# linebender/vello

Measured on AMD Instinct MI355X. Metric: frames/sec paris-30k 1600x1600 MSAA16; scenes/sec at 1/2/4/8 GPU, higher is better.
Workload: dtype f32+u32

## Files before the change

### vello_amd/csrc/engine/coarse.hip

```cpp
#include "engine.h"

namespace vk {

namespace {

constexpr uint32_t SUB_W = 8;
#ifndef VK_COARSE_NW
#define VK_COARSE_NW 8
#endif
constexpr uint32_t NW = VK_COARSE_NW;
constexpr uint32_t WG = 64 * NW;
constexpr uint32_t NB = 64 * NW;
constexpr uint32_t QCAP = 2 * NB;
static_assert((QCAP & (QCAP - 1u)) == 0u && QCAP >= NB - 1u + WG, "the queue is a ring of a power of two that holds a batch's leftovers and a round's arrivals");
constexpr uint32_t PART_CHUNK = 256;
constexpr uint32_t NONE = 0xffffffffu;
constexpr uint32_t EMIT_GROUP = 8;
constexpr uint32_t INITIAL_ROOM = PTCL_INITIAL_ALLOC - 1u - 2u - 1u;
constexpr uint32_t REGION_SLACK = 62u;
constexpr uint32_t KIND_NONE = 0u, KIND_PATH2 = 1u, KIND_PATH3 = 2u, KIND_BEGIN = 3u;

typedef unsigned long long u64;

struct __attribute__((packed, aligned(4))) PtclWords2 { uint32_t a, b; };
// ... 41 lines not shown
    if (k >= c) { k -= c; w >>= 4; pos += 4u; }
    c = (uint32_t)__popc(w & 3u);
    if (k >= c) { k -= c; w >>= 2; pos += 2u; }
    if (k >= (w & 1u)) pos += 1u;
    return pos;
}

__device__ __forceinline__ u64 transpose64(u64 x, uint32_t lane) {
    const u64 masks[6] = {0x00000000ffffffffull, 0x0000ffff0000ffffull, 0x00ff00ff00ff00ffull,
                          0x0f0f0f0f0f0f0f0full, 0x3333333333333333ull, 0x5555555555555555ull};
#pragma unroll
    for (uint32_t s = 0; s < 6u; s++) {
        const uint32_t j = 32u >> s;
        const u64 mask = masks[s];
        const uint32_t olo = (uint32_t)__shfl_xor((int)(uint32_t)x, (int)j), ohi = (uint32_t)__shfl_xor((int)(uint32_t)(x >> 32), (int)j);
        const u64 other = make64(olo, ohi);
        if ((lane & j) == 0u) x = (x & mask) | ((other & mask) << j);
        else x = (x & ~mask) | ((other & ~mask) >> j);
    }
    return x;
}

__device__ __forceinline__ uint32_t words_of(u64 m, u64 g, u64 k1, u64 k2, u64 k3) {
    return 3u * popc64(g) + 3u * popc64(m & k1) + 4u * popc64(m & k2) + popc64(m & k3);
}

__device__ __forceinline__ PtclWords2 plane_window(const uint32_t *__restrict__ bits, uint32_t b) {
    return *reinterpret_cast<const PtclWords2 *>(bits + (b >> 3));
}
__device__ __forceinline__ uint32_t window_bits(PtclWords2 w, uint32_t byte_shift, uint32_t b) {
    return (((w.a >> byte_shift) & 0xffu) | (((w.b >> byte_shift) & 0xffu) << 8)) >> (b & 7u);
}

}

__global__ void __launch_bounds__(256) k_coarse_prep(Config cfg, uint32_t n_el_blocks, const uint32_t *__restrict__ scene,
                                                     const DrawMonoid *__restrict__ draw_monoids, const uint32_t *__restrict__ info_bin_data,
                                                     const Path *__restrict__ paths, const Tile *__restrict__ tiles, const Bump *__restrict__ bump,
                                                     CoarseEl *__restrict__ coarse_el, uint32_t *__restrict__ tile_bits) {
    const uint32_t tid = threadIdx.x;
    if (blockIdx.x < n_el_blocks) {
        const uint32_t drawobj_ix = blockIdx.x * 256u + tid;
        if (drawobj_ix >= cfg.layout.n_draw_objects) return;
        CoarseEl e;
        e.tag = scene[cfg.layout.draw_tag_base + drawobj_ix];
        e.flags = 0u; e.w0 = 0u; e.dd = 0u; e.di = 0u; e.tiles = 0u; e.bbox_x = 0u; e.bbox_y = 0u;
        if (e.tag != DRAWTAG_NOP) {
            const DrawMonoid dm = draw_monoids[drawobj_ix];
            e.dd = cfg.layout.draw_data_base + dm.scene_offset;
            e.di = dm.info_offset;
            e.flags = info_bin_data[dm.info_offset];
            e.w0 = scene[e.dd];
            const Path path = paths[dm.path_ix];
            e.tiles = path.tiles;
            e.bbox_x = path.bbox[0] | (path.bbox[2] << 16);
            e.bbox_y = path.bbox[1] | (path.bbox[3] << 16);
        }
        coarse_el[drawobj_ix] = e;
        return;
    }
    const uint32_t n_tiles = minu(bump->tile, cfg.tiles_size);
    const uint32_t lane = tid & 63u;
    const uint32_t wave = (blockIdx.x - n_el_blocks) * 4u + (tid >> 6);
    const uint32_t n_waves = (gridDim.x - n_el_blocks) * 4u;
    for (uint32_t chunk = wave; chunk * 64u < n_tiles; chunk += n_waves) {
        const uint32_t i = chunk * 64u + lane;
        Tile t{1, 0u};
        if (i < n_tiles) t = tiles[i];
        const unsigned long long ms = __ballot(t.segment_count_or_ix != 0u);
        const unsigned long long mz = __ballot(t.backdrop == 0);
        const unsigned long long mo = __ballot((t.backdrop & 1) == 0);
        if (lane < 8u) {
            const uint32_t sh = 8u * lane;
            tile_bits[(size_t)chunk * 8u + lane] = ((uint32_t)(ms >> sh) & 0xffu) | (((uint32_t)(mz >> sh) & 0xffu) << 8) | (((uint32_t)(mo >> sh) & 0xffu) << 16);
        }
    }
}


__global__ void __launch_bounds__(WG) k_coarse(Config cfg, const uint32_t *__restrict__ scene, const BinHeader *__restrict__ bin_headers,
                                                const uint32_t *__restrict__ info_bin_data, const CoarseEl *__restrict__ coarse_el,
                                                const uint32_t *__restrict__ tile_bits, Tile *tiles, Bump *bump,
                                                uint32_t *ptcl, bool allow_cull, uint32_t *work_count, uint32_t *tile_order,
                                                SliceItem *slice_items, uint32_t *slice_counters, uint32_t slice_cap, uint32_t cov_cap,
                                                uint32_t slice_fills, uint32_t slice_min_fills) {
#ifdef VELLO_SIMT_EMU
    __shared__ CoarseLds sh;
#else
    extern __shared__ __attribute__((aligned(16))) unsigned char coarse_lds_raw[];
    CoarseLds &sh = *reinterpret_cast<CoarseLds *>(coarse_lds_raw);
#endif
    const uint32_t tid = threadIdx.x;
    const uint32_t lane = tid & 63u, wave = tid >> 6;
    {
        uint32_t failed = bump->failed & (STAGE_BINNING | STAGE_TILE_ALLOC | STAGE_FLATTEN | FAILED_SCENE);
        if (bump->seg_counts > cfg.seg_counts_size) failed |= STAGE_PATH_COUNT;
        if (failed != 0u) {
            if (blockIdx.x == 0 && tid == 0) atomicOr(&bump->failed, failed);
            return;
        }
    }
    const uint32_t width_in_bins = (cfg.width_in_tiles + N_TILE_X - 1u) / N_TILE_X;
    const uint32_t height_in_bins = (cfg.height_in_tiles + N_TILE_Y - 1u) / N_TILE_Y;
    const uint32_t n_bins = width_in_bins * height_in_bins;
    const uint32_t bin_ix = ((blockIdx.x >> 3) >> 2) * 8u + (blockIdx.x & 7u);
    const uint32_t quad = (blockIdx.x >> 3) & 3u;
    if (bin_ix >= n_bins) return;
    const uint32_t aligned_n_bins = (n_bins + N_TILE - 1u) & ~(N_TILE - 1u);
    const uint32_t n_partitions = (cfg.layout.n_draw_objects + N_TILE - 1u) / N_TILE;
    const uint32_t sub_x0 = N_TILE_X * (bin_ix % width_in_bins) + SUB_W * (quad & 1u);
    const uint32_t sub_y0 = N_TILE_Y * (bin_ix / width_in_bins) + SUB_W * (quad >> 1);
    const bool has_clips = cfg.layout.n_clips != 0u;
    const bool cull = allow_cull && !has_clips;
    const uint32_t ptcl_dyn_start = cfg.width_in_tiles * cfg.height_in_tiles * PTCL_INITIAL_ALLOC;
    if (tid == 0u) sh.seg_arrive = 0u;
#ifdef VELLO_COARSE_PROF
    long long prof_prev = clock64();
    uint32_t prof_acc[16] = {0u, 0u, 0u, 0u, 0u, 0u, 0u, 0u, 0u, 0u, 0u, 0u, 0u, 0u, 0u, 0u};
#define CPROF(k) do { const long long t_ = clock64(); prof_acc[k] += (uint32_t)(t_ - prof_prev); prof_prev = t_; } while (0)
#define CPROF_COUNT(k) prof_acc[k] += 1u
#else
#define CPROF(k)
#define CPROF_COUNT(k)
#endif

    const uint32_t this_tile_ix = (sub_y0 + lane / SUB_W) * cfg.width_in_tiles + sub_x0 + lane % SUB_W;
    const uint32_t blend_offset = this_tile_ix * PTCL_INITIAL_ALLOC;
    const uint32_t list_start = blend_offset + 1u;
    uint32_t cur = list_start;
    uint32_t room = INITIAL_ROOM;
    bool dead = false;
    uint32_t words_total = 0u;
    uint32_t fills_total = 0u;
    uint32_t clip_zero_depth = 0u, clip_depth = 0u, render_blend_depth = 0u, max_blend_depth = 0u;

    uint32_t partition_ix = 0u;
    uint32_t chunk_total = 0u, chunk_pos = 0u;
    auto refill = [&]() {
        __syncthreads();
        if (wave == 0u) {
            uint32_t carry = 0u;
#pragma unroll
            for (uint32_t k = 0; k < PART_CHUNK / 64u; k++) {
                const uint32_t p = partition_ix + k * 64u + lane;
                uint32_t count = 0u, off = 0u;
                if (p < n_partitions) {
                    const BinHeader bh = bin_headers[(size_t)p * aligned_n_bins + bin_ix];
                    count = bh.element_count;
                    off = bh.chunk_offset;
                }
                const uint32_t incl = wave_incl_scan_u32(count, (int)lane) + carry;
                sh.part_end[k * 64u + lane] = incl;
                sh.part_off[k * 64u + lane] = off;
                carry = (uint32_t)__shfl((int)incl, 63);
            }
            if (lane == 0u) sh.bcast = carry;
        }
        __syncthreads();
        chunk_total = sh.bcast;
        chunk_pos = 0u;
        partition_ix += PART_CHUNK;
    };
    auto fetch_index = [&](uint32_t &d) -> bool {
        while (chunk_pos >= chunk_total && partition_ix < n_partitions) refill();
        const bool any = chunk_pos < chunk_total;
        const uint32_t ix = chunk_pos + tid;
        d = NONE;
        if (ix < chunk_total) {
            uint32_t part = 0u;
#pragma unroll
            for (uint32_t i = 0; i < 8u; i++) {
                const uint32_t probe = part + (128u >> i);
                if (ix >= sh.part_end[probe - 1u]) part = probe;
            }
            const uint32_t local = ix - (part > 0u ? sh.part_end[part - 1u] : 0u);
            d = info_bin_data[cfg.layout.bin_data_start + sh.part_off[part] + local];
        }
        chunk_pos = minu(chunk_pos + WG, chunk_total);
        return any;
    };

    uint32_t qh = 0u, qlen = 0u;
    auto load_el = [&](uint32_t d) -> CoarseEl {
        CoarseEl e;
        e.tag = DRAWTAG_NOP;
        e.flags = 0u; e.w0 = 0u; e.dd = 0u; e.di = 0u; e.tiles = 0u; e.bbox_x = 0u; e.bbox_y = 0u;
        if (d != NONE) {
            const uint4 *p = reinterpret_cast<const uint4 *>(coarse_el + d);
            const uint4 a = p[0], b = p[1];
            e.tag = a.x; e.flags = a.y; e.w0 = a.z; e.dd = a.w;
            e.di = b.x; e.tiles = b.y; e.bbox_x = b.z; e.bbox_y = b.w;
        }
        return e;
    };
    uint32_t d_next;
    bool cur_valid = fetch_index(d_next);
    CoarseEl el_next = load_el(d_next);
    bool next_valid = cur_valid ? fetch_index(d_next) : false;
    bool more = cur_valid;
    while (cur_valid || qlen > 0u) {
        if (cur_valid) {
            const CoarseEl el = el_next;
            if (next_valid) el_next = load_el(d_next);
            const bool nn_valid = next_valid ? fetch_index(d_next) : false;
            cur_valid = next_valid;
            next_valid = nn_valid;
            more = cur_valid;
            CPROF(8);
            const int32_t bx0 = (int32_t)(el.bbox_x & 0xffffu), bx1 = (int32_t)(el.bbox_x >> 16);
            const int32_t by0 = (int32_t)(el.bbox_y & 0xffffu), by1 = (int32_t)(el.bbox_y >> 16);
            const int32_t dx = bx0 - (int32_t)sub_x0, dy = by0 - (int32_t)sub_y0;
            const int32_t x0 = clampi(dx, 0, (int32_t)SUB_W), y0 = clampi(dy, 0, (int32_t)SUB_W);
            const int32_t x1 = clampi(bx1 - (int32_t)sub_x0, 0, (int32_t)SUB_W), y1 = clampi(by1 - (int32_t)sub_y0, 0, (int32_t)SUB_W);
            const bool meets = el.tag != DRAWTAG_NOP && x1 > x0 && y1 > y0;
            const uint32_t stride = (uint32_t)(bx1 - bx0);
            const uint32_t base = el.tiles - (uint32_t)(dy * (int32_t)stride + dx);
            u64 inc = 0ull, kil = 0ull, seg = 0ull, clr = 0ull;
            {
                const uint32_t rx0 = (uint32_t)x0, ry0 = (uint32_t)y0;
                const uint32_t w = meets ? (uint32_t)(x1 - x0) : 0u, h = meets ? (uint32_t)(y1 - y0) : 0u;
                const bool is_clip = (el.tag & 1u) != 0u;
                const uint32_t BLEND_CLIP = (128u << 8) | 3u;
                const bool is_blend = is_clip && el.w0 != BLEND_CLIP;
                const bool even_odd = (el.flags & DRAW_INFO_FLAGS_FILL_RULE_BIT) != 0u;
                const uint32_t clear_byte = even_odd ? 16u : 8u;
                const uint32_t wmask = (1u << w) - 1u;
                const uint32_t b0 = base + stride * ry0 + rx0;
                PtclWords2 win[SUB_W];
#pragma unroll
                for (uint32_t r = 0; r < SUB_W; r++) win[r] = plane_window(tile_bits, r < h ? b0 + stride * r : 0u);
#pragma unroll
                for (uint32_t r = 0; r < SUB_W; r++) {
                    const uint32_t rmask = r < h ? wmask : 0u;
                    const uint32_t b = b0 + stride * r;
                    const uint32_t sg = window_bits(win[r], 0u, b) & rmask;
                    const uint32_t clear = window_bits(win[r], clear_byte, b) & rmask;
                    const uint32_t in = is_blend ? rmask : (sg | ((is_clip ? clear : ~clear) & rmask));
                    const uint32_t shift = ((ry0 + r) * SUB_W + rx0) & 63u;
                    inc |= (u64)in << shift;
                    seg |= (u64)(in & sg) << shift;
                    clr |= (u64)(in & clear) << shift;
                }
                if (cull && el.tag == DRAWTAG_FILL_COLOR && (el.w0 >> 24) == 0xffu) kil = inc & ~seg;
            }
            const bool keep = inc != 0ull;
            const u64 m = __ballot(keep);
            CPROF(9);
            if (lane == 0u) sh.wave_cnt[wave] = popc64(m);
            __syncthreads();
            CPROF(10);
            uint32_t before = 0u, total_new = 0u;
#pragma unroll
            for (uint32_t w = 0; w < NW; w++) {
                const uint32_t c = sh.wave_cnt[w];
                if (w < wave) before += c;
                total_new += c;
            }
            if (keep) {
                const uint32_t q = (qh + qlen + before + popc64(m & below64(lane))) & (QCAP - 1u);
                uint32_t kind = KIND_NONE;
                switch (el.tag) {
                case DRAWTAG_FILL_COLOR: case DRAWTAG_FILL_IMAGE: kind = KIND_PATH2; break;
                case DRAWTAG_BLURRED_ROUNDED_RECT: case DRAWTAG_FILL_LIN_GRADIENT: case DRAWTAG_FILL_RAD_GRADIENT:
                case DRAWTAG_FILL_SWEEP_GRADIENT: case DRAWTAG_END_CLIP: kind = KIND_PATH3; break;
                case DRAWTAG_BEGIN_CLIP: kind = KIND_BEGIN; break;
                default: break;
                }
                sh.tag[q] = el.tag;
                sh.flags[q] = el.flags;
                sh.w0[q] = el.w0;
                sh.dd[q] = el.dd;
                sh.di[q] = el.di;
                sh.stride[q] = stride;
                sh.base[q] = base;
                sh.kind[q] = kind;
                sh.cover[q][0] = (uint32_t)inc; sh.cover[q][1] = (uint32_t)(inc >> 32);
                sh.cover[q][2] = (uint32_t)kil; sh.cover[q][3] = (uint32_t)(kil >> 32);
                sh.cover[q][4] = (uint32_t)seg; sh.cover[q][5] = (uint32_t)(seg >> 32);
                sh.cover[q][6] = (uint32_t)clr; sh.cover[q][7] = (uint32_t)(clr >> 32);
            }
            qlen += total_new;
            __syncthreads();
            CPROF(0);
            CPROF_COUNT(6);
        }

        while (qlen >= NB || (!more && qlen > 0u)) {
            const uint32_t n = minu(qlen, NB);
            const uint32_t cnt = n > wave * 64u ? minu(n - wave * 64u, 64u) : 0u;
            const uint32_t q0 = qh + wave * 64u;
            const uint32_t my_kind = lane < cnt ? (sh.kind[(q0 + lane) & (QCAP - 1u)]) : KIND_NONE;
            const u64 k1 = __ballot(my_kind == KIND_PATH2), k2 = __ballot(my_kind == KIND_PATH3), k3 = __ballot(my_kind == KIND_BEGIN);
            const u64 k_end = has_clips ? __ballot(lane < cnt && sh.tag[(q0 + lane) & (QCAP - 1u)] == DRAWTAG_END_CLIP) : 0ull;
            u64 inc = 0ull, seg = 0ull, clr = 0ull, kil = 0ull;
            if (lane < cnt) {
                const uint32_t *c = sh.cover[(q0 + lane) & (QCAP - 1u)];
                inc = make64(c[0], c[1]);
                if (cull) kil = make64(c[2], c[3]);
                seg = make64(c[4], c[5]);
                if (has_clips) clr = make64(c[6], c[7]);
            }
            inc = transpose64(inc, lane);
            seg = transpose64(seg, lane);
            if (cull) kil = transpose64(kil, lane);
            if (has_clips) clr = transpose64(clr, lane);
            const uint32_t klast = kil != 0ull ? 64u - (uint32_t)__clzll((long long)kil) : 0u;
            sh.kslice[wave][lane] = klast;
            if (has_clips) {
                sh.em[wave][lane][0] = (uint32_t)inc; sh.em[wave][lane][1] = (uint32_t)(inc >> 32);
                sh.gm[wave][lane][0] = (uint32_t)seg; sh.gm[wave][lane][1] = (uint32_t)(seg >> 32);
                sh.cl[wave][lane][0] = (uint32_t)clr; sh.cl[wave][lane][1] = (uint32_t)(clr >> 32);
                if (lane == 0u) {
                    sh.kinds[wave][0][0] = (uint32_t)k3; sh.kinds[wave][0][1] = (uint32_t)(k3 >> 32);
                    sh.kinds[wave][1][0] = (uint32_t)k_end; sh.kinds[wave][1][1] = (uint32_t)(k_end >> 32);
                }
            }
            __syncthreads();
            bool tile_killed = false;
            if (cull) {
                bool later = false;
#pragma unroll
                for (uint32_t w = 0; w < NW; w++) {
                    const uint32_t kl = sh.kslice[w][lane];
                    tile_killed = tile_killed || kl != 0u;
                    if (w > wave && kl != 0u) later = true;
                }
                if (later) inc = 0ull;
                else if (klast != 0u) inc &= ~below64(klast - 1u);
            }
            if (has_clips) {
                if (wave == 0u) {
#pragma unroll 1
                    for (uint32_t w = 0; w < NW; w++) {
                        const u64 m = make64(sh.em[w][lane][0], sh.em[w][lane][1]);
                        const u64 sg = make64(sh.gm[w][lane][0], sh.gm[w][lane][1]);
                        const u64 cr = make64(sh.cl[w][lane][0], sh.cl[w][lane][1]);
                        const u64 kb = make64(sh.kinds[w][0][0], sh.kinds[w][0][1]);
                        const u64 ke = make64(sh.kinds[w][1][0], sh.kinds[w][1][1]);
                        u64 clipbits = m & (kb | ke);
                        u64 act = 0ull;
// ... 41 lines not shown
            const u64 gmask = seg & em & (k1 | k2);
            const uint32_t n_pairs_t = popc64(em);
            const uint32_t pair_incl = wave_incl_scan_u32(n_pairs_t, (int)lane);
            const uint32_t total_pairs = (uint32_t)__shfl((int)pair_incl, 63);
            sh.em[wave][lane][0] = (uint32_t)em; sh.em[wave][lane][1] = (uint32_t)(em >> 32);
            sh.gm[wave][lane][0] = (uint32_t)gmask; sh.gm[wave][lane][1] = (uint32_t)(gmask >> 32);
            sh.pend[wave][lane] = pair_incl;
            sh.S[wave][lane] = words_of(em, gmask, k1, k2, k3) | (popc64(gmask) << 16);
            wave_lds_sync();
            const uint32_t n_iter = (total_pairs + 63u) / 64u;
            auto pair_of = [&](uint32_t p, uint32_t &t, uint32_t &b, bool &has_segs) {
                t = 0u;
#pragma unroll
                for (uint32_t i = 0; i < 6u; i++) {
                    const uint32_t probe = t + (32u >> i);
                    if (p >= sh.pend[wave][probe - 1u]) t = probe;
                }
                const uint32_t k = p - (t > 0u ? sh.pend[wave][t - 1u] : 0u);
                const u64 m = make64(sh.em[wave][t][0], sh.em[wave][t][1]);
                b = kth_bit64(m, k);
                has_segs = ((make64(sh.gm[wave][t][0], sh.gm[wave][t][1]) >> b) & 1ull) != 0ull;
            };
            auto load_group = [&](uint32_t g0, uint32_t (&info)[EMIT_GROUP], uint32_t (&tix)[EMIT_GROUP], Tile (&tl)[EMIT_GROUP]) {
#pragma unroll
                for (uint32_t u = 0; u < EMIT_GROUP; u++) {
                    const uint32_t p = (g0 + u) * 64u + lane;
                    info[u] = 0u;
                    tix[u] = 0u;
                    tl[u] = Tile{0, 0u};
                    if (g0 + u < n_iter && p < total_pairs) {
                        uint32_t t, b;
                        bool has_segs;
                        pair_of(p, t, b, has_segs);
                        const uint32_t q = (q0 + b) & (QCAP - 1u);
                        tix[u] = sh.base[q] + sh.stride[q] * (t / SUB_W) + (t % SUB_W);
                        info[u] = t | (b << 8) | (has_segs ? 1u << 16 : 0u) | (1u << 17);
                        if (has_segs) tl[u] = tiles[tix[u]];
                    }
                }
            };
            uint32_t info[EMIT_GROUP], tix[EMIT_GROUP];
            Tile tl[EMIT_GROUP];
            load_group(0u, info, tix, tl);
            __syncthreads();
            CPROF(1);
            if (wave == 0u) {
                uint32_t s_w[NW], W = 0u, n_fill = 0u;
#pragma unroll
                for (uint32_t w = 0; w < NW; w++) {
                    const uint32_t s = sh.S[w][lane];
                    s_w[w] = s & 0xffffu;
                    W += s_w[w];
                    n_fill += s >> 16;
                }
                if (tile_killed && !dead) {
                    cur = list_start;
                    room = INITIAL_ROOM;
                    words_total = 0u;
                    fills_total = 0u;
                }
                words_total += W;
                fills_total += n_fill;
                const bool need = W > room && !dead;
                const uint32_t rsize = need ? W + 2u + REGION_SLACK : 0u;
                const uint32_t r_incl = wave_incl_scan_u32(rsize, (int)lane);
                const uint32_t r_total = (uint32_t)__shfl((int)r_incl, 63);
                uint32_t r_base = 0u;
                if (lane == 0u && r_total != 0u) r_base = atomicAdd(&bump->ptcl, r_total);
                r_base = (uint32_t)__shfl((int)r_base, 0);
                if (need) {
                    const uint32_t start = ptcl_dyn_start + r_base + (r_incl - rsize);
                    if (start < ptcl_dyn_start || start + rsize > cfg.ptcl_size || start + rsize < start) {
                        atomicOr(&bump->failed, STAGE_COARSE);
                        dead = true;
                    } else {
                        *reinterpret_cast<PtclWords2 *>(ptcl + cur) = PtclWords2{CMD_JUMP, start};
                        cur = start;
                        room = W + REGION_SLACK;
                    }
                }
                uint32_t wb = dead ? NONE : cur;
#pragma unroll
                for (uint32_t w = 0; w < NW; w++) {
                    sh.wordbase[w][lane] = wb;
                    if (!dead) wb += s_w[w];
                }
                if (!dead) {
                    cur += W;
                    room -= W;
                }
            }
            CPROF(2);
            uint32_t seg_first;
            {
                uint32_t my_segs = 0u;
#pragma unroll
                for (uint32_t u = 0; u < EMIT_GROUP; u++) my_segs += tl[u].segment_count_or_ix;
                const uint32_t seg_incl = wave_incl_scan_u32(my_segs, (int)lane);
                const uint32_t seg_total = (uint32_t)__shfl((int)seg_incl, 63);
                uint32_t arrived = 0u;
                if (lane == 0u) {
                    sh.seg_tot[wave] = seg_total;
#ifdef VELLO_SIMT_EMU
                    arrived = atomicAdd(&sh.seg_arrive, 1u);
#else
                    arrived = __hip_atomic_fetch_add(&sh.seg_arrive, 1u, __ATOMIC_ACQ_REL, __HIP_MEMORY_SCOPE_WORKGROUP);
#endif
                }
                arrived = (uint32_t)__shfl((int)arrived, 0);
                if (arrived == NW - 1u) {
                    const uint32_t tot = lane < NW ? sh.seg_tot[lane] : 0u;
                    const uint32_t incl = wave_incl_scan_u32(tot, (int)lane);
                    const uint32_t all = (uint32_t)__shfl((int)incl, 63);
                    uint32_t got = 0u;
                    if (lane == 0u && all != 0u) got = atomicAdd(&bump->segments, all);
                    got = (uint32_t)__shfl((int)got, 0);
                    if (lane < NW) sh.seg_base[lane] = got + (incl - tot);
                    if (lane == 0u) sh.seg_arrive = 0u;
                }
                __syncthreads();
                seg_first = sh.seg_base[wave] + (seg_incl - my_segs);
            }
            for (uint32_t g0 = 0; g0 < n_iter; g0 += EMIT_GROUP) {
                uint32_t seg_next = seg_first;
                if (g0 != 0u) {
                    load_group(g0, info, tix, tl);
                    uint32_t my_segs = 0u;
#pragma unroll
                    for (uint32_t u = 0; u < EMIT_GROUP; u++) my_segs += tl[u].segment_count_or_ix;
                    const uint32_t seg_incl = wave_incl_scan_u32(my_segs, (int)lane);
                    const uint32_t seg_total = (uint32_t)__shfl((int)seg_incl, 63);
                    uint32_t got = 0u;
                    if (lane == 0u && seg_total != 0u) got = atomicAdd(&bump->segments, seg_total);
                    seg_next = (uint32_t)__shfl((int)got, 0) + (seg_incl - my_segs);
                }
#pragma unroll
                for (uint32_t u = 0; u < EMIT_GROUP; u++) {
                    if ((info[u] >> 17) == 0u) continue;
                    const uint32_t t = info[u] & 0xffu, b = (info[u] >> 8) & 0xffu;
                    const bool has_segs = ((info[u] >> 16) & 1u) != 0u;
                    const uint32_t n_segs = tl[u].segment_count_or_ix;
                    const uint32_t seg_ix = seg_next;
                    seg_next += n_segs;
                    const uint32_t wbase = sh.wordbase[wave][t];
                    if (wbase == NONE) continue;
                    const uint32_t q = (q0 + b) & (QCAP - 1u);
                    const u64 m = make64(sh.em[wave][t][0], sh.em[wave][t][1]);
                    const u64 g = make64(sh.gm[wave][t][0], sh.gm[wave][t][1]);
                    const u64 bel = below64(b);
                    uint32_t off = wbase + words_of(m & bel, g & bel, k1, k2, k3);
                    const uint32_t tag = sh.tag[q];
                    if (tag == DRAWTAG_BEGIN_CLIP) {
                        ptcl[off] = CMD_BEGIN_CLIP;
                        continue;
                    }
                    const uint32_t draw_flags = sh.flags[q];
                    if (has_segs) {
                        tiles[tix[u]].segment_count_or_ix = ~seg_ix;
                        const uint32_t even_odd = (draw_flags & DRAW_INFO_FLAGS_FILL_RULE_BIT) != 0u ? 1u : 0u;
                        *reinterpret_cast<PtclWords4 *>(ptcl + off) = PtclWords4{CMD_FILL, (n_segs << 1) | even_odd, seg_ix, (uint32_t)tl[u].backdrop};
                        off += 4u;
                    } else {
                        ptcl[off] = CMD_SOLID;
                        off += 1u;
                    }
                    const uint32_t w0 = sh.w0[q], di = sh.di[q];
                    switch (tag) {
                    case DRAWTAG_FILL_COLOR: *reinterpret_cast<PtclWords2 *>(ptcl + off) = PtclWords2{CMD_COLOR, w0}; break;
                    case DRAWTAG_FILL_IMAGE: *reinterpret_cast<PtclWords2 *>(ptcl + off) = PtclWords2{CMD_IMAGE, di + 1u}; break;
                    case DRAWTAG_BLURRED_ROUNDED_RECT: *reinterpret_cast<PtclWords3 *>(ptcl + off) = PtclWords3{CMD_BLUR_RECT, di + 1u, w0}; break;
                    case DRAWTAG_FILL_LIN_GRADIENT: *reinterpret_cast<PtclWords3 *>(ptcl + off) = PtclWords3{CMD_LIN_GRAD, w0, di + 1u}; break;
                    case DRAWTAG_FILL_RAD_GRADIENT: *reinterpret_cast<PtclWords3 *>(ptcl + off) = PtclWords3{CMD_RAD_GRAD, w0, di + 1u}; break;
                    case DRAWTAG_FILL_SWEEP_GRADIENT: *reinterpret_cast<PtclWords3 *>(ptcl + off) = PtclWords3{CMD_SWEEP_GRAD, w0, di + 1u}; break;
                    case DRAWTAG_END_CLIP: *reinterpret_cast<PtclWords3 *>(ptcl + off) = PtclWords3{CMD_END_CLIP, w0, scene[sh.dd[q] + 1u]}; break;
                    default: break;
                    }
                }
            }
            CPROF(3);
            qh = (qh + n) & (QCAP - 1u);
            qlen -= n;
            __syncthreads();
            CPROF(4);
            CPROF_COUNT(7);
        }
    }
    if (wave == 0u) {
        const bool in_target = sub_x0 + lane % SUB_W < cfg.width_in_tiles && sub_y0 + lane / SUB_W < cfg.height_in_tiles;
        if (in_target) {
            if (!dead) ptcl[cur] = CMD_END;
            uint32_t blend_ix = 0u;
            if (max_blend_depth > BLEND_STACK_SPLIT) {
                uint32_t scratch_size = (max_blend_depth - BLEND_STACK_SPLIT) * TILE_WIDTH * TILE_HEIGHT;
                blend_ix = atomicAdd(&bump->blend, scratch_size);
                if (blend_ix + scratch_size > cfg.blend_size) atomicOr(&bump->failed, STAGE_COARSE);
            }
            ptcl[blend_offset] = blend_ix;
            ptcl[blend_offset + PTCL_INITIAL_ALLOC - 1u] = words_total;
        }
        const uint32_t n_tiles = cfg.width_in_tiles * cfg.height_in_tiles;
        uint32_t bucket = in_target ? minu(FINE_WORK_BUCKETS - 1u, words_total / FINE_BUCKET_WORDS) : NONE;
        uint32_t n_sl = 0u;
        if (in_target && !dead && slice_min_fills != 0u && fills_total >= slice_min_fills) n_sl = minu((fills_total + slice_fills - 1u) / slice_fills, 0xffffu);
        if (__ballot(n_sl != 0u) != 0ull) {
            const uint32_t cov_need = n_sl != 0u ? n_sl * slice_fills * 64u + 64u : 0u;
            const uint32_t it_incl = wave_incl_scan_u32(n_sl, (int)lane), cv_incl = wave_incl_scan_u32(cov_need, (int)lane);
            uint32_t it_base = 0u, cv_base = 0u;
            if (lane == 63u) {
                it_base = atomicAdd(&work_count[FINE_WORK_BUCKETS], it_incl);
                cv_base = atomicAdd(&work_count[FINE_WORK_BUCKETS + 1u], cv_incl);
            }
            it_base = (uint32_t)__shfl((int)it_base, 63) + (it_incl - n_sl);
            cv_base = (uint32_t)__shfl((int)cv_base, 63) + (cv_incl - cov_need);
            if (n_sl != 0u) {
                const bool fits = it_base + n_sl <= slice_cap && it_base + n_sl >= it_base && cv_base + cov_need <= cov_cap && cv_base + cov_need >= cv_base;
                for (uint32_t k = 0; k < n_sl && it_base + k < slice_cap && it_base + k >= it_base; k++)
                    slice_items[it_base + k] = SliceItem{fits ? this_tile_ix : ~0u, k | (n_sl << 16), cv_base, it_base};
                if (fits) {
                    slice_counters[it_base] = 0u;
                    bucket = NONE;
                }
            }
        }
        static_assert(FINE_WORK_BUCKETS <= 64u, "a lane per bucket");
        uint32_t my_count = 0u, my_rank = 0u;
        for (uint32_t bk = 0; bk < FINE_WORK_BUCKETS; bk++) {
            const u64 m = __ballot(bucket == bk);
            if (lane == bk) my_count = popc64(m);
            if (bucket == bk) my_rank = popc64(m & below64(lane));
        }
        uint32_t base = 0u;
        if (lane < FINE_WORK_BUCKETS && my_count != 0u) base = atomicAdd(&work_count[lane], my_count);
        base = (uint32_t)__shfl((int)base, (int)(bucket & 63u));
        if (bucket != NONE) {
            const uint32_t pos = base + my_rank;
            if (pos < n_tiles) tile_order[bucket * n_tiles + pos] = this_tile_ix;
        }
    }
#ifdef VELLO_COARSE_PROF
    CPROF(5);
    if (tid == 0u && cfg.ptcl_size >= 8192u && blockIdx.x < 512u)
        for (uint32_t k = 0; k < 16u; k++) ptcl[cfg.ptcl_size - 8192u + blockIdx.x * 16u + k] = prof_acc[k];
#endif
}

int enable_coarse_lds() {
#ifndef VELLO_SIMT_EMU
    return (int)hipFuncSetAttribute(reinterpret_cast<const void *>(k_coarse), hipFuncAttributeMaxDynamicSharedMemorySize, (int)sizeof(CoarseLds));
#else
    return 0;
#endif
}

constexpr uint32_t COARSE_GRID_BINS = 8u;
uint32_t coarse_batch_draws() { return NB; }
uint32_t coarse_grid_bins() { return COARSE_GRID_BINS; }

void launch_coarse(const Frame &f, hipStream_t s, hipEvent_t *mid) {
    const uint32_t wb = (f.cfg.width_in_tiles + 15u) / 16u, hb = (f.cfg.height_in_tiles + 15u) / 16u;
    if (wb * hb == 0) {
        if (mid) (void)hipEventRecord(mid[0], s);
        return;
    }
    const uint32_t n_el_blocks = (f.cfg.layout.n_draw_objects + DRAW_WG - 1u) / DRAW_WG;
    uint32_t n_bit_blocks = (uint32_t)(((uint64_t)f.cfg.tiles_size + 256u * 8u - 1u) / (256u * 8u));
    if (n_bit_blocks > 2048u) n_bit_blocks = 2048u;
    if (n_bit_blocks < 1u) n_bit_blocks = 1u;
    hipLaunchKernelGGL(k_coarse_prep, dim3(n_el_blocks + n_bit_blocks), dim3(256), 0, s, dd_config(f), n_el_blocks, f.scene, f.draw_monoids,
                       f.info_bin_data, f.paths, f.tiles, f.bump(), f.coarse_el, f.tile_bits);
    if (mid) (void)hipEventRecord(mid[0], s);
    const uint32_t n_wg = ((wb * hb + COARSE_GRID_BINS - 1u) / COARSE_GRID_BINS) * COARSE_GRID_BINS * 4u;
    hipLaunchKernelGGL(k_coarse, dim3(n_wg), dim3(WG), sizeof(CoarseLds), s, f.cfg, f.scene, f.bin_headers, f.info_bin_data, f.coarse_el, f.tile_bits,
                       f.tiles, f.bump(), f.ptcl, !f.no_cull, f.control->work_count, f.tile_order,
                       f.slice_items, f.slice_counters, f.slice_cap, f.cov_cap, f.slice_fills, f.slice_min_fills);
}

}
```

### vello_amd/csrc/engine/engine.h

```cpp
#pragma once
#include <cstddef>
#include "common.h"

namespace vk {

constexpr uint32_t SCAN_STATUS_AGG = 1, SCAN_STATUS_PREFIX = 2;
constexpr uint32_t PATHTAG_PART_WORDS = 1024;
constexpr uint32_t DRAW_PART = 256;
constexpr uint32_t DRAW_WG = 256;
#ifndef VK_FLATTEN_TPT
#define VK_FLATTEN_TPT 4
#endif
constexpr uint32_t FLATTEN_TAGS_PER_THREAD = VK_FLATTEN_TPT;
constexpr uint32_t FLATTEN_BLOCK_TAGS = 256 * FLATTEN_TAGS_PER_THREAD;
#ifndef VK_PC_LPT
#define VK_PC_LPT 4
#endif
constexpr uint32_t PATH_COUNT_LINES_PER_THREAD = VK_PC_LPT;
constexpr uint32_t PATH_COUNT_CHUNK = 256 * PATH_COUNT_LINES_PER_THREAD;
constexpr int64_t PATH_COUNT_SMALL_MAX_LINES = 768 * 256;
constexpr uint32_t SPIN_LIMIT = 1u << 24;
constexpr uint32_t FAILED_INTERNAL = 0x80000000u;
constexpr uint32_t FAILED_SCENE = 0x40000000u;
constexpr uint32_t FINE_WORK_BUCKETS = 32;
// ... 15 lines not shown
#endif
constexpr uint32_t FINE_SLICE_FILLS_IN_FLIGHT = VK_SLICE_FILLS_IN_FLIGHT, FINE_SLICE_MIN_FILLS_IN_FLIGHT = VK_SLICE_MIN_FILLS_IN_FLIGHT;
constexpr uint32_t FINE_SLICE_FILLS_FORCED = 4, FINE_SLICE_MIN_FILLS_FORCED = 5;
struct SliceItem {
    uint32_t tile_ix;
    uint32_t k_and_n;
    uint32_t cov_base;
    uint32_t first_item;
};
constexpr uint32_t CLIP_PART = 256;
constexpr uint32_t CLIP_MAX_PARTS = 2048;
struct ClipEl { uint32_t clip_ix; float x0, y0, x1, y1; };
__host__ __device__ inline uint32_t clip_parts_pad(uint32_t parts) {
    uint32_t n = 2u;
    while (n < parts) n <<= 1;
    return n;
}
inline size_t clip_scratch_words(uint32_t n_clips) {
    size_t parts = (n_clips + CLIP_PART - 1u) / CLIP_PART;
    size_t par = parts * (CLIP_PART * 5u + 4u + 2u + 1u) + 2u * (size_t)clip_parts_pad((uint32_t)parts);
    size_t seq = ((size_t)n_clips + 1u) * 6u;
    return par > seq ? par : seq;
}

struct Control {
    Bump bump;
    uint32_t ticket_pathtag;
    uint32_t ticket_draw;
    uint32_t heavy_count[4];
    uint32_t pad[2];
    uint32_t work_count[FINE_WORK_BUCKETS];
    uint32_t slice_items;
    uint32_t cov_words;
    uint32_t pad2[48 - FINE_WORK_BUCKETS - 2];
    uint32_t arc_count[64];
};
static_assert(sizeof(Control) == 512, "Control");
static_assert(offsetof(Control, slice_items) == offsetof(Control, work_count) + 4u * FINE_WORK_BUCKETS, "Control::slice_items follows work_count");
static_assert(offsetof(Control, cov_words) == offsetof(Control, slice_items) + 4u, "Control::cov_words follows slice_items");
constexpr uint32_t FLATTEN_ARC_SHARDS = 64;
#ifndef VK_STROKES_GRID_SIDE_BY_SIDE
#define VK_STROKES_GRID_SIDE_BY_SIDE 4096u
#endif
#ifndef VK_STROKES_GRID_OWN_LAUNCH
#define VK_STROKES_GRID_OWN_LAUNCH 384u
#endif
inline uint32_t flatten_strokes_grid(uint32_t n_seg_max, bool side_by_side) {
    const uint32_t cap = side_by_side ? VK_STROKES_GRID_SIDE_BY_SIDE : VK_STROKES_GRID_OWN_LAUNCH;
    const uint32_t g = (n_seg_max + 255u) / 256u;
    return g > cap ? cap : (g < 1u ? 1u : g);
}
inline uint32_t flatten_arc_shard_cap(uint32_t n_seg_max, bool side_by_side) {
    const uint32_t grid = flatten_strokes_grid(n_seg_max, side_by_side);
    const uint32_t rounds = ((n_seg_max + 255u) / 256u + grid - 1u) / grid;
    return ((grid + FLATTEN_ARC_SHARDS - 1u) / FLATTEN_ARC_SHARDS) * (rounds < 1u ? 1u : rounds) * 256u;
}

struct Frame {
    Config cfg;
    uint32_t n_tag_words;
    uint32_t n_scene_words;
    uint32_t aa;
    const uint32_t *scene;
    uint32_t xf_base;
    bool has_view;
    Xform view;
    bool retained;
    const uint32_t *xf_owner;
    const uint32_t *pose_words;
    uint32_t n_instances;
    hipStream_t pose_stream;
    hipEvent_t pose_mark;
    bool pose_check;
// ... 233 lines not shown
```

### vello_amd/csrc/engine/fine.hip

```cpp
#include "engine.h"

namespace vk {

namespace {

constexpr uint32_t PIXELS_PER_THREAD = 4;
constexpr int GRADIENT_WIDTH = 512;
constexpr uint32_t LUMINANCE_MASK_LAYER = 0x10000u;

enum {
    FP_INTERP = 0,
    FP_BATCH_SCAN,
    FP_BATCH_SEGS,
    FP_BATCH_ITEMS,
    FP_FILL_APPLY,
    FP_FILL_PREFIX,
    FP_FILL_SPARSE,
    FP_FILL_RESTORE,
    FP_FILL_EVENODD,
    FP_FILL_UNBATCHED,
    FP_BLEND,
    FP_RARE,
    FP_RARE_END_CLIP,
    FP_RARE_GRAD,
// ... 1489 lines not shown
        slice_n = it.k_and_n >> 16;
        mode = MODE_COV;
        fill_lo = k * slice_fills;
        fill_hi = k + 1u == slice_n ? 0xffffffffu : (k + 1u) * slice_fills;
        fill_room = slice_n * slice_fills;
        cov_base = it.cov_base;
        first_item = it.first_item;
    } else {
        const uint32_t rest = blockIdx.x - (AA != 0 ? slice_blocks : 0u);
        static_assert(FINE_WORK_BUCKETS <= 64u, "a lane per bucket");
        const uint32_t cnt = lane < FINE_WORK_BUCKETS ? minu(work_count[FINE_WORK_BUCKETS - 1u - lane], n_tiles) : 0u;
        const uint32_t incl = wave_incl_scan_u32(cnt, (int)lane);
        const unsigned long long beyond = __ballot(incl > rest);
        if (beyond == 0ull) return;
        const uint32_t bl = (uint32_t)__ffsll((long long)beyond) - 1u;
        const uint32_t slot = (FINE_WORK_BUCKETS - 1u - bl) * n_tiles + (rest - wave_read(incl - cnt, bl));
        tile_ix = (uint32_t)__builtin_amdgcn_readfirstlane((int)tile_order[slot]);
        if (tile_ix >= n_tiles) return;
    }
    const uint32_t tile_x = tile_ix % cfg.width_in_tiles, tile_y = tile_ix / cfg.width_in_tiles;
    const float xy_x = (float)(tile_x * TILE_WIDTH + lx * PIXELS_PER_THREAD);
    const float xy_y = (float)(tile_y * TILE_HEIGHT + ly);
    vec4 rgba[4];
    uint32_t blend_stack[BLEND_STACK_SPLIT][4];
    uint32_t clip_depth;
    float area[4];
    uint32_t cmd_ix;
    uint32_t win_base;
    uint32_t win;
    auto rd = [&](uint32_t ix) -> uint32_t {
        return (uint32_t)__builtin_amdgcn_readlane((int)win, (int)__builtin_amdgcn_readfirstlane((int)(ix - win_base)));
    };
    auto ensure = [&](uint32_t ix, uint32_t n_words) {
        if (ix + n_words > win_base + FINE_WINDOW_WORDS) {
            win_base = ix;
            uint32_t a = win_base + lane;
            win = a < cfg.ptcl_size ? ptcl[a] : 0u;
        }
    };
    FineProf prof;
    prof.start();
    FineTimeline tl;
    tl.start();
    uint32_t blend_offset;
    constexpr float COV_SCALE = AA == 2 ? 0.0625f : 0.125f;
    uint32_t fill_no = 0u;
    auto start_list = [&]() {
        const vec4 base_color = unpack4x8unorm(cfg.base_color);
#pragma unroll
        for (int i = 0; i < 4; i++) {
            rgba[i] = base_color;
            area[i] = 0.0f;
        }
        clip_depth = 0u;
        cmd_ix = tile_ix * PTCL_INITIAL_ALLOC;
        win_base = cmd_ix;
        win = ptcl[win_base + lane];
        blend_offset = rd(cmd_ix);
        cmd_ix += 1u;
        fill_no = 0u;
    };
    auto store_cov = [&]() {
        uint32_t b = 0u;
#pragma unroll
        for (uint32_t i = 0; i < 4u; i++) b |= (uint32_t)(area[i] * (1.0f / COV_SCALE)) << (8u * i);
        if (fill_no < fill_room) __hip_atomic_store(&cov[cov_base + fill_no * 64u + lane], b, __ATOMIC_RELAXED, __HIP_MEMORY_SCOPE_AGENT);
        fill_no += 1u;
// ... 291 lines not shown
```

Measured before the change: 2673.

## Walk draw objects back-to-front in coarse to stop at opaque-covered tiles

Adds a back-to-front coarse mode, selected when culling is allowed, there are no clips, and the prep kernel flagged at least one opaque solid fill. Partitions and queue batches are processed in reverse order, and per-tile command lists are built backwards through prepended regions linked by jumps. Each tile stops once an opaque fill covers it, and the workgroup exits early once all its tiles are covered, so occluded draws are never binned or emitted. The cost is extra prep-kernel sync and flag writes, a templated second kernel path, and the fine window reloading on backward jumps. The chained, non-contiguous command lists may also hurt fine's read locality.

```diff
diff --git a/vello_amd/csrc/engine/coarse.hip b/vello_amd/csrc/engine/coarse.hip
--- a/vello_amd/csrc/engine/coarse.hip
+++ b/vello_amd/csrc/engine/coarse.hip
@@ -97,31 +97,42 @@
     return (((w.a >> byte_shift) & 0xffu) | (((w.b >> byte_shift) & 0xffu) << 8)) >> (b & 7u);
 }
 
+__device__ __forceinline__ bool coarse_back_to_front(bool allow_cull, uint32_t n_clips, bool opaque_fills) {
+    return allow_cull && n_clips == 0u && opaque_fills;
+}
+
 }
 
 __global__ void __launch_bounds__(256) k_coarse_prep(Config cfg, uint32_t n_el_blocks, const uint32_t *__restrict__ scene,
                                                      const DrawMonoid *__restrict__ draw_monoids, const uint32_t *__restrict__ info_bin_data,
                                                      const Path *__restrict__ paths, const Tile *__restrict__ tiles, const Bump *__restrict__ bump,
-                                                     CoarseEl *__restrict__ coarse_el, uint32_t *__restrict__ tile_bits) {
+                                                     CoarseEl *__restrict__ coarse_el, uint32_t *__restrict__ tile_bits, uint32_t *opaque_fills) {
     const uint32_t tid = threadIdx.x;
     if (blockIdx.x < n_el_blocks) {
+        __shared__ uint32_t any_opaque;
+        if (tid == 0u) any_opaque = 0u;
+        __syncthreads();
         const uint32_t drawobj_ix = blockIdx.x * 256u + tid;
-        if (drawobj_ix >= cfg.layout.n_draw_objects) return;
-        CoarseEl e;
-        e.tag = scene[cfg.layout.draw_tag_base + drawobj_ix];
-        e.flags = 0u; e.w0 = 0u; e.dd = 0u; e.di = 0u; e.tiles = 0u; e.bbox_x = 0u; e.bbox_y = 0u;
-        if (e.tag != DRAWTAG_NOP) {
-            const DrawMonoid dm = draw_monoids[drawobj_ix];
-            e.dd = cfg.layout.draw_data_base + dm.scene_offset;
-            e.di = dm.info_offset;
-            e.flags = info_bin_data[dm.info_offset];
-            e.w0 = scene[e.dd];
-            const Path path = paths[dm.path_ix];
-            e.tiles = path.tiles;
-            e.bbox_x = path.bbox[0] | (path.bbox[2] << 16);
-            e.bbox_y = path.bbox[1] | (path.bbox[3] << 16);
-        }
-        coarse_el[drawobj_ix] = e;
+        if (drawobj_ix < cfg.layout.n_draw_objects) {
+            CoarseEl e;
+            e.tag = scene[cfg.layout.draw_tag_base + drawobj_ix];
+            e.flags = 0u; e.w0 = 0u; e.dd = 0u; e.di = 0u; e.tiles = 0u; e.bbox_x = 0u; e.bbox_y = 0u;
+            if (e.tag != DRAWTAG_NOP) {
+                const DrawMonoid dm = draw_monoids[drawobj_ix];
+                e.dd = cfg.layout.draw_data_base + dm.scene_offset;
+                e.di = dm.info_offset;
+                e.flags = info_bin_data[dm.info_offset];
+                e.w0 = scene[e.dd];
+                const Path path = paths[dm.path_ix];
+                e.tiles = path.tiles;
+                e.bbox_x = path.bbox[0] | (path.bbox[2] << 16);
+                e.bbox_y = path.bbox[1] | (path.bbox[3] << 16);
+            }
+            coarse_el[drawobj_ix] = e;
+            if (e.tag == DRAWTAG_FILL_COLOR && (e.w0 >> 24) == 0xffu) any_opaque = 1u;
+        }
+        __syncthreads();
+        if (tid == 0u && any_opaque != 0u) opaque_fills[blockIdx.x % COARSE_OPAQUE_SHARDS] = 1u;
         return;
     }
     const uint32_t n_tiles = minu(bump->tile, cfg.tiles_size);
@@ -143,18 +154,13 @@
 }
 
 
-__global__ void __launch_bounds__(WG) k_coarse(Config cfg, const uint32_t *__restrict__ scene, const BinHeader *__restrict__ bin_headers,
+template <bool B2F>
+__device__ __forceinline__ void coarse_workgroup(CoarseLds &sh, const Config &cfg, const uint32_t *__restrict__ scene, const BinHeader *__restrict__ bin_headers,
                                                 const uint32_t *__restrict__ info_bin_data, const CoarseEl *__restrict__ coarse_el,
                                                 const uint32_t *__restrict__ tile_bits, Tile *tiles, Bump *bump,
                                                 uint32_t *ptcl, bool allow_cull, uint32_t *work_count, uint32_t *tile_order,
                                                 SliceItem *slice_items, uint32_t *slice_counters, uint32_t slice_cap, uint32_t cov_cap,
                                                 uint32_t slice_fills, uint32_t slice_min_fills) {
-#ifdef VELLO_SIMT_EMU
-    __shared__ CoarseLds sh;
-#else
-    extern __shared__ __attribute__((aligned(16))) unsigned char coarse_lds_raw[];
-    CoarseLds &sh = *reinterpret_cast<CoarseLds *>(coarse_lds_raw);
-#endif
     const uint32_t tid = threadIdx.x;
     const uint32_t lane = tid & 63u, wave = tid >> 6;
     {
@@ -175,8 +181,8 @@
     const uint32_t n_partitions = (cfg.layout.n_draw_objects + N_TILE - 1u) / N_TILE;
     const uint32_t sub_x0 = N_TILE_X * (bin_ix % width_in_bins) + SUB_W * (quad & 1u);
     const uint32_t sub_y0 = N_TILE_Y * (bin_ix / width_in_bins) + SUB_W * (quad >> 1);
-    const bool has_clips = cfg.layout.n_clips != 0u;
-    const bool cull = allow_cull && !has_clips;
+    const bool has_clips = !B2F && cfg.layout.n_clips != 0u;
+    const bool cull = B2F || (allow_cull && !has_clips);
     const uint32_t ptcl_dyn_start = cfg.width_in_tiles * cfg.height_in_tiles * PTCL_INITIAL_ALLOC;
     if (tid == 0u) sh.seg_arrive = 0u;
 #ifdef VELLO_COARSE_PROF
@@ -198,11 +204,16 @@
     uint32_t words_total = 0u;
     uint32_t fills_total = 0u;
     uint32_t clip_zero_depth = 0u, clip_depth = 0u, render_blend_depth = 0u, max_blend_depth = 0u;
-
-    uint32_t partition_ix = 0u;
+    bool covered = B2F && !(sub_x0 + lane % SUB_W < cfg.width_in_tiles && sub_y0 + lane / SUB_W < cfg.height_in_tiles);
+    u64 covered_mask = B2F ? __ballot(covered) : 0ull;
+    uint32_t head = NONE, front = 0u;
+    bool finished = false;
+
+    uint32_t partition_ix = B2F ? ((n_partitions + PART_CHUNK - 1u) / PART_CHUNK) * PART_CHUNK : 0u;
     uint32_t chunk_total = 0u, chunk_pos = 0u;
     auto refill = [&]() {
         __syncthreads();
+        if (B2F) partition_ix -= PART_CHUNK;
         if (wave == 0u) {
             uint32_t carry = 0u;
 #pragma unroll
@@ -224,12 +235,12 @@
         __syncthreads();
         chunk_total = sh.bcast;
         chunk_pos = 0u;
-        partition_ix += PART_CHUNK;
+        if (!B2F) partition_ix += PART_CHUNK;
     };
     auto fetch_index = [&](uint32_t &d) -> bool {
-        while (chunk_pos >= chunk_total && partition_ix < n_partitions) refill();
+        while (chunk_pos >= chunk_total && (B2F ? partition_ix > 0u : partition_ix < n_partitions)) refill();
         const bool any = chunk_pos < chunk_total;
-        const uint32_t ix = chunk_pos + tid;
+        const uint32_t ix = B2F ? chunk_total - 1u - (chunk_pos + tid) : chunk_pos + tid;
         d = NONE;
         if (ix < chunk_total) {
             uint32_t part = 0u;
@@ -263,7 +274,8 @@
     CoarseEl el_next = load_el(d_next);
     bool next_valid = cur_valid ? fetch_index(d_next) : false;
     bool more = cur_valid;
-    while (cur_valid || qlen > 0u) {
+    bool all_covered = false;
+    while ((cur_valid || qlen > 0u) && !all_covered) {
         if (cur_valid) {
             const CoarseEl el = el_next;
             if (next_valid) el_next = load_el(d_next);
@@ -306,6 +318,7 @@
                     seg |= (u64)(in & sg) << shift;
                     clr |= (u64)(in & clear) << shift;
                 }
+                if (B2F) inc &= ~covered_mask;
                 if (cull && el.tag == DRAWTAG_FILL_COLOR && (el.w0 >> 24) == 0xffu) kil = inc & ~seg;
             }
             const bool keep = inc != 0ull;
@@ -353,13 +366,15 @@
         while (qlen >= NB || (!more && qlen > 0u)) {
             const uint32_t n = minu(qlen, NB);
             const uint32_t cnt = n > wave * 64u ? minu(n - wave * 64u, 64u) : 0u;
-            const uint32_t q0 = qh + wave * 64u;
-            const uint32_t my_kind = lane < cnt ? (sh.kind[(q0 + lane) & (QCAP - 1u)]) : KIND_NONE;
+            auto slot_q = [&](uint32_t j) -> uint32_t { return (B2F ? qh + n - 1u - j : qh + j) & (QCAP - 1u); };
+            const uint32_t j0 = wave * 64u;
+            const bool last_batch = B2F && !more && qlen <= NB;
+            const uint32_t my_kind = lane < cnt ? (sh.kind[slot_q(j0 + lane)]) : KIND_NONE;
             const u64 k1 = __ballot(my_kind == KIND_PATH2), k2 = __ballot(my_kind == KIND_PATH3), k3 = __ballot(my_kind == KIND_BEGIN);
-            const u64 k_end = has_clips ? __ballot(lane < cnt && sh.tag[(q0 + lane) & (QCAP - 1u)] == DRAWTAG_END_CLIP) : 0ull;
+            const u64 k_end = has_clips ? __ballot(lane < cnt && sh.tag[slot_q(j0 + lane)] == DRAWTAG_END_CLIP) : 0ull;
             u64 inc = 0ull, seg = 0ull, clr = 0ull, kil = 0ull;
             if (lane < cnt) {
-                const uint32_t *c = sh.cover[(q0 + lane) & (QCAP - 1u)];
+                const uint32_t *c = sh.cover[slot_q(j0 + lane)];
                 inc = make64(c[0], c[1]);
                 if (cull) kil = make64(c[2], c[3]);
                 seg = make64(c[4], c[5]);
@@ -371,6 +386,7 @@
             if (has_clips) clr = transpose64(clr, lane);
             const uint32_t klast = kil != 0ull ? 64u - (uint32_t)__clzll((long long)kil) : 0u;
             sh.kslice[wave][lane] = klast;
+            if (B2F && covered) inc = 0ull;
             if (has_clips) {
                 sh.em[wave][lane][0] = (uint32_t)inc; sh.em[wave][lane][1] = (uint32_t)(inc >> 32);
                 sh.gm[wave][lane][0] = (uint32_t)seg; sh.gm[wave][lane][1] = (uint32_t)(seg >> 32);
@@ -478,7 +494,7 @@
                         uint32_t t, b;
                         bool has_segs;
                         pair_of(p, t, b, has_segs);
-                        const uint32_t q = (q0 + b) & (QCAP - 1u);
+                        const uint32_t q = slot_q(j0 + b);
                         tix[u] = sh.base[q] + sh.stride[q] * (t / SUB_W) + (t % SUB_W);
                         info[u] = t | (b << 8) | (has_segs ? 1u << 16 : 0u) | (1u << 17);
                         if (has_segs) tl[u] = tiles[tix[u]];
@@ -499,7 +515,7 @@
                     W += s_w[w];
                     n_fill += s >> 16;
                 }
-                if (tile_killed && !dead) {
+                if (!B2F && tile_killed && !dead) {
                     cur = list_start;
                     room = INITIAL_ROOM;
                     words_total = 0u;
@@ -507,8 +523,11 @@
                 }
                 words_total += W;
                 fills_total += n_fill;
-                const bool need = W > room && !dead;
-                const uint32_t rsize = need ? W + 2u + REGION_SLACK : 0u;
+                const bool live = B2F && !covered && !dead;
+                const bool fin = live && (tile_killed || last_batch);
+                const bool in_block = fin && W <= INITIAL_ROOM;
+                const bool need = B2F ? live && !in_block && W > front : W > room && !dead;
+                const uint32_t rsize = need ? W + 2u + (fin ? 0u : REGION_SLACK) : 0u;
                 const uint32_t r_incl = wave_incl_scan_u32(rsize, (int)lane);
                 const uint32_t r_total = (uint32_t)__shfl((int)r_incl, 63);
                 uint32_t r_base = 0u;
@@ -519,19 +538,38 @@
                     if (start < ptcl_dyn_start || start + rsize > cfg.ptcl_size || start + rsize < start) {
                         atomicOr(&bump->failed, STAGE_COARSE);
                         dead = true;
+                    } else if (B2F) {
+                        const uint32_t at = start + (rsize - 2u - W);
+                        *reinterpret_cast<PtclWords2 *>(ptcl + at + W) = head == NONE ? PtclWords2{CMD_END, 0u} : PtclWords2{CMD_JUMP, head};
+                        head = at;
+                        front = rsize - 2u - W;
                     } else {
                         *reinterpret_cast<PtclWords2 *>(ptcl + cur) = PtclWords2{CMD_JUMP, start};
                         cur = start;
                         room = W + REGION_SLACK;
                     }
-                }
-                uint32_t wb = dead ? NONE : cur;
+                } else if (in_block) {
+                    *reinterpret_cast<PtclWords2 *>(ptcl + list_start + W) = head == NONE ? PtclWords2{CMD_END, 0u} : PtclWords2{CMD_JUMP, head};
+                    head = list_start;
+                    front = 0u;
+                } else if (live) {
+                    head -= W;
+                    front -= W;
+                }
+                if (B2F) {
+                    if (fin && !dead) {
+                        if (!in_block) *reinterpret_cast<PtclWords2 *>(ptcl + list_start) = head == NONE ? PtclWords2{CMD_END, 0u} : PtclWords2{CMD_JUMP, head};
+                        finished = true;
+                    }
+                    cur = head;
+                }
+                uint32_t wb = (dead || (B2F && !live)) ? NONE : cur;
 #pragma unroll
                 for (uint32_t w = 0; w < NW; w++) {
                     sh.wordbase[w][lane] = wb;
-                    if (!dead) wb += s_w[w];
-                }
-                if (!dead) {
+                    if (wb != NONE) wb += s_w[w];
+                }
+                if (!B2F && !dead) {
                     cur += W;
                     room -= W;
                 }
@@ -590,7 +628,7 @@
                     seg_next += n_segs;
                     const uint32_t wbase = sh.wordbase[wave][t];
                     if (wbase == NONE) continue;
-                    const uint32_t q = (q0 + b) & (QCAP - 1u);
+                    const uint32_t q = slot_q(j0 + b);
                     const u64 m = make64(sh.em[wave][t][0], sh.em[wave][t][1]);
                     const u64 g = make64(sh.gm[wave][t][0], sh.gm[wave][t][1]);
                     const u64 bel = below64(b);
@@ -629,12 +667,22 @@
             __syncthreads();
             CPROF(4);
             CPROF_COUNT(7);
+            if (B2F) {
+                covered = covered || tile_killed || last_batch;
+                covered_mask = __ballot(covered);
+                if (covered_mask == ~0ull) {
+                    all_covered = true;
+                    break;
+                }
+            }
         }
     }
     if (wave == 0u) {
         const bool in_target = sub_x0 + lane % SUB_W < cfg.width_in_tiles && sub_y0 + lane / SUB_W < cfg.height_in_tiles;
         if (in_target) {
-            if (!dead) ptcl[cur] = CMD_END;
+            if (B2F) {
+                if (!dead && !finished) *reinterpret_cast<PtclWords2 *>(ptcl + list_start) = head == NONE ? PtclWords2{CMD_END, 0u} : PtclWords2{CMD_JUMP, head};
+            } else if (!dead) ptcl[cur] = CMD_END;
             uint32_t blend_ix = 0u;
             if (max_blend_depth > BLEND_STACK_SPLIT) {
                 uint32_t scratch_size = (max_blend_depth - BLEND_STACK_SPLIT) * TILE_WIDTH * TILE_HEIGHT;
@@ -690,6 +738,27 @@
 #endif
 }
 
+__global__ void __launch_bounds__(WG) k_coarse(Config cfg, const uint32_t *__restrict__ scene, const BinHeader *__restrict__ bin_headers,
+                                                const uint32_t *__restrict__ info_bin_data, const CoarseEl *__restrict__ coarse_el,
+                                                const uint32_t *__restrict__ tile_bits, Tile *tiles, Bump *bump,
+                                                uint32_t *ptcl, bool allow_cull, const uint32_t *__restrict__ opaque_fills, uint32_t *work_count,
+                                                uint32_t *tile_order, SliceItem *slice_items, uint32_t *slice_counters, uint32_t slice_cap,
+                                                uint32_t cov_cap, uint32_t slice_fills, uint32_t slice_min_fills) {
+#ifdef VELLO_SIMT_EMU
+    __shared__ CoarseLds sh;
+#else
+    extern __shared__ __attribute__((aligned(16))) unsigned char coarse_lds_raw[];
+    CoarseLds &sh = *reinterpret_cast<CoarseLds *>(coarse_lds_raw);
+#endif
+    const uint32_t my_shard = (threadIdx.x & 63u) < COARSE_OPAQUE_SHARDS ? opaque_fills[threadIdx.x & 63u] : 0u;
+    if (coarse_back_to_front(allow_cull, cfg.layout.n_clips, __ballot(my_shard != 0u) != 0ull))
+        coarse_workgroup<true>(sh, cfg, scene, bin_headers, info_bin_data, coarse_el, tile_bits, tiles, bump, ptcl, allow_cull, work_count, tile_order, slice_items,
+                               slice_counters, slice_cap, cov_cap, slice_fills, slice_min_fills);
+    else
+        coarse_workgroup<false>(sh, cfg, scene, bin_headers, info_bin_data, coarse_el, tile_bits, tiles, bump, ptcl, allow_cull, work_count, tile_order, slice_items,
+                                slice_counters, slice_cap, cov_cap, slice_fills, slice_min_fills);
+}
+
 int enable_coarse_lds() {
 #ifndef VELLO_SIMT_EMU
     return (int)hipFuncSetAttribute(reinterpret_cast<const void *>(k_coarse), hipFuncAttributeMaxDynamicSharedMemorySize, (int)sizeof(CoarseLds));
@@ -713,11 +782,11 @@
     if (n_bit_blocks > 2048u) n_bit_blocks = 2048u;
     if (n_bit_blocks < 1u) n_bit_blocks = 1u;
     hipLaunchKernelGGL(k_coarse_prep, dim3(n_el_blocks + n_bit_blocks), dim3(256), 0, s, dd_config(f), n_el_blocks, f.scene, f.draw_monoids,
-                       f.info_bin_data, f.paths, f.tiles, f.bump(), f.coarse_el, f.tile_bits);
+                       f.info_bin_data, f.paths, f.tiles, f.bump(), f.coarse_el, f.tile_bits, f.control->opaque_fills);
     if (mid) (void)hipEventRecord(mid[0], s);
     const uint32_t n_wg = ((wb * hb + COARSE_GRID_BINS - 1u) / COARSE_GRID_BINS) * COARSE_GRID_BINS * 4u;
     hipLaunchKernelGGL(k_coarse, dim3(n_wg), dim3(WG), sizeof(CoarseLds), s, f.cfg, f.scene, f.bin_headers, f.info_bin_data, f.coarse_el, f.tile_bits,
-                       f.tiles, f.bump(), f.ptcl, !f.no_cull, f.control->work_count, f.tile_order,
+                       f.tiles, f.bump(), f.ptcl, !f.no_cull, f.control->opaque_fills, f.control->work_count, f.tile_order,
                        f.slice_items, f.slice_counters, f.slice_cap, f.cov_cap, f.slice_fills, f.slice_min_fills);
 }
 
diff --git a/vello_amd/csrc/engine/engine.h b/vello_amd/csrc/engine/engine.h
--- a/vello_amd/csrc/engine/engine.h
+++ b/vello_amd/csrc/engine/engine.h
@@ -71,13 +71,16 @@
     uint32_t work_count[FINE_WORK_BUCKETS];
     uint32_t slice_items;
     uint32_t cov_words;
-    uint32_t pad2[48 - FINE_WORK_BUCKETS - 2];
+    uint32_t opaque_fills[8];
+    uint32_t pad2[48 - FINE_WORK_BUCKETS - 2 - 8];
     uint32_t arc_count[64];
 };
 static_assert(sizeof(Control) == 512, "Control");
 static_assert(offsetof(Control, slice_items) == offsetof(Control, work_count) + 4u * FINE_WORK_BUCKETS, "Control::slice_items follows work_count");
 static_assert(offsetof(Control, cov_words) == offsetof(Control, slice_items) + 4u, "Control::cov_words follows slice_items");
 constexpr uint32_t FLATTEN_ARC_SHARDS = 64;
+constexpr uint32_t COARSE_OPAQUE_SHARDS = 8;
+static_assert(sizeof(Control::opaque_fills) == 4u * COARSE_OPAQUE_SHARDS, "Control::opaque_fills");
 #ifndef VK_STROKES_GRID_SIDE_BY_SIDE
 #define VK_STROKES_GRID_SIDE_BY_SIDE 4096u
 #endif
diff --git a/vello_amd/csrc/engine/fine.hip b/vello_amd/csrc/engine/fine.hip
--- a/vello_amd/csrc/engine/fine.hip
+++ b/vello_amd/csrc/engine/fine.hip
@@ -1545,7 +1545,7 @@
         return (uint32_t)__builtin_amdgcn_readlane((int)win, (int)__builtin_amdgcn_readfirstlane((int)(ix - win_base)));
     };
     auto ensure = [&](uint32_t ix, uint32_t n_words) {
-        if (ix + n_words > win_base + FINE_WINDOW_WORDS) {
+        if (ix + n_words > win_base + FINE_WINDOW_WORDS || ix < win_base) {
             win_base = ix;
             uint32_t a = win_base + lane;
             win = a < cfg.ptcl_size ? ptcl[a] : 0u;
```

New measurement: 2791, median of 6. 1.04x the previous value.
